# wjf5203/VNext

Hardware: AMD Instinct MI355X
Metric: MSDeformAttn fwd+bwd Gpoints/s (T=5,L=4,Q=300,H=8,K=4) (higher is better)
Workload: dtype f32; 1 GPU; SeqFormer-R50 T=5 360p clip folded to B=5: MSDeformAttn decoder call, Lq=300, S=5100, M=8, D=32, L=4, K=4, loc~U[0,1); 1 step = fwd+bwd; input_rotation_sets=12, parallelism=dp1 (clips sharded, no data-path collective)

## Files before the change

### vnext_amd/csrc/msda_d32_gvdirect_body.h

```cpp
#pragma once
#include <type_traits>

#include "msda_gv_common.h"

namespace vnx {
namespace rec {

#ifndef VNX_GVD_UNITS_PER_CU
#define VNX_GVD_UNITS_PER_CU 3
#endif
#ifndef VNX_GVD_PARTS
#define VNX_GVD_PARTS 2
#endif
#ifndef VNX_GVD_AUX
#define VNX_GVD_AUX 0
#endif
#ifndef VNX_GVD_ABL
#define VNX_GVD_ABL 0
#endif
#ifndef VNX_GVD_FULL_BARRIERS
#define VNX_GVD_FULL_BARRIERS 0
#endif


#ifdef VNX_GVD_STAMPS
static __device__ unsigned long long g_gvd_stamps[4096 * 8];
#define VNX_GVD_STAMP(k) do { if (tid == 0 && vblock < 4096) g_gvd_stamps[vblock * 8 + (k)] = (unsigned long long)wall_clock64(); } while (0)
#else
#define VNX_GVD_STAMP(k) do { } while (0)
#endif

constexpr int kGvdQc = VNX_GVD_QC;
constexpr int kGvdRows = VNX_GVD_ROWS;
constexpr int kGvdSamples = kGvdQc * 4;
constexpr int kGvdSpt = (kGvdSamples + kThreads - 1) / kThreads;
constexpr int kGvdCap = 4 * kGvdSamples;
constexpr int kGvdParts = VNX_GVD_PARTS;
constexpr int kGvdPartPieces = 8 / kGvdParts;
constexpr int kGvdRowPieces = (kGvdQc * kGvdPartPieces + kThreads - 1) / kThreads;
constexpr size_t kGvdLdsBytes = size_t(kGvdQc) * 16 * kGvdPartPieces + size_t(kGvdCap) * 6 + size_t(kGvdRows) * 4 + 16 + 4 * kLevelsMax * 4;
static_assert(kGvdParts == 1 || kGvdParts == 2, "whole rows or halves");
static_assert(kGvdLdsBytes * VNX_GVD_UNITS_PER_CU <= 160 * 1024, "the units that share a CU must fit its LDS");
static_assert(kGvdCap < 65536 && kGvdQc < 65536, "tap ranks and query slots fit 16 bits");

template <typename TV, typename TL, int P_T>
__device__ __forceinline__ void msda_bwd_gv_direct_body(const int64_t* __restrict__ shapes, const int64_t* __restrict__ lsi,
                                                        const TL* __restrict__ loc, const TL* __restrict__ attn,
                                                        const TV* __restrict__ grad_out, TV* __restrict__ grad_value,
                                                        const MsdaDims& d, int ut, int rows_max, int compact, unsigned long long* stamps,
                                                        uint32_t vblock, unsigned char* smem) {
  stamp_begin(stamps);
  constexpr int D = 32;
  float4_t* grows = reinterpret_cast<float4_t*>(smem);
  float* l_wt = reinterpret_cast<float*>(grows + kGvdQc * kGvdPartPieces);
  uint32_t* cnt = reinterpret_cast<uint32_t*>(l_wt + kGvdCap);
  uint32_t* alloc = cnt + kGvdRows;
  int* meta = reinterpret_cast<int*>(alloc + 4);
  uint16_t* l_slot = reinterpret_cast<uint16_t*>(meta + 4 * kLevelsMax);

  const int P = P_T > 0 ? P_T : d.P;
  const int tid = threadIdx.x, lane = tid & 63;
  int rest, b, m;
  if (kGvPair16 && sizeof(TV) == 2 && (d.M & 1) == 0) gv_decode_block<true>(vblock, d.M, d.B, rest, b, m);
  else gv_decode_block<false>(vblock, d.M, d.B, rest, b, m);
  const int unit = rest / d.B;
  VNX_GVD_STAMP(0);

  const TV* go_head = grad_out + (int64_t(b) * d.Lq * d.M + m) * D;
  const uint32_t q_stride = uint32_t(d.M) * uint32_t(D);
  constexpr uint32_t kOutOfRange = 0x80000000u;
  const __amdgpu_buffer_rsrc_t go_src = uniform_rsrc(go_head, uint32_t(d.Lq) * q_stride * uint32_t(sizeof(TV)));
  int qc = kGvdSamples / P;
  qc = qc < kGvdQc ? qc : kGvdQc;
  float4_t pg[kGvdParts][kGvdRowPieces];
  auto request_rows = [&](int q_lo) {
    const int tg = opaque(tid);
#pragma unroll
    for (int part = 0; part < kGvdParts; ++part) {
#pragma unroll
      for (int i = 0; i < kGvdRowPieces; ++i) {
        const int g = i * kThreads + tg, ql = g / kGvdPartPieces;
        const bool ok = ql < qc && q_lo + ql < d.Lq;
        const uint32_t off = ok ? (__umul24(uint32_t(q_lo + ql), q_stride) + uint32_t(part * kGvdPartPieces + g % kGvdPartPieces) * 4u) * uint32_t(sizeof(TV))
                                : kOutOfRange;
        pg[part][i] = load4_buf<TV>(go_src, off);
      }
    }
  };
  auto stage_rows = [&](int part) {
    const int tg = opaque(tid);
#pragma unroll
    for (int i = 0; i < kGvdRowPieces; ++i)
      if ((i * kThreads + tg) / kGvdPartPieces < kGvdQc) grows[i * kThreads + tg] = pg[part][i];
  };
  int lvl = -1, r0 = 0, r1 = 0, Hl = 0, Wl = 0, start = 0, gshift = 0;
  bool packed = true;
  if (tid < d.L) {
    const int H = int(shapes[2 * tid]), W = int(shapes[2 * tid + 1]), first = int(lsi[tid]);
    const GvdSplit sp = gvd_level_split(H * W, ut, d.Lq, P, rows_max);
    meta[4 * tid] = H; meta[4 * tid + 1] = W; meta[4 * tid + 2] = first;
    meta[4 * tid + 3] = sp.units | (sp.rpu << 18) | (sp.gshift << 29);
  }
  for (int i = tid; i < kGvdRows; i += kThreads) cnt[i] = 0;
  if (tid == 0) alloc[0] = 0;
  lds_barrier();
  {
    int running = 0;
    int u = unit;
    for (int l = 0; l < d.L; ++l) {
      packed = packed && (meta[4 * l + 2] == running);
      running += meta[4 * l] * meta[4 * l + 1];
    }
    for (int l = d.L - 1; l >= 0; --l) {
      const int H = meta[4 * l], W = meta[4 * l + 1], st = meta[4 * l + 2];
      const uint32_t ur = uint32_t(meta[4 * l + 3]);
      const int n = H * W, units = int(ur & 0x3ffffu), rpu = int((ur >> 18) & 0x7ffu);
      if (lvl < 0) {
        if (u < units) {
          lvl = l; Hl = H; Wl = W; start = st; gshift = int(ur >> 29);
          r0 = u * rpu;
          r1 = r0 + rpu < n ? r0 + rpu : n;
        } else {
          u -= units;
        }
      }
    }
    packed = packed && (running == d.S);
  }
  if (!packed || lvl < 0) {
    return;
  }
  lvl = __builtin_amdgcn_readfirstlane(lvl); r0 = __builtin_amdgcn_readfirstlane(r0); r1 = __builtin_amdgcn_readfirstlane(r1);
  Hl = __builtin_amdgcn_readfirstlane(Hl); Wl = __builtin_amdgcn_readfirstlane(Wl); start = __builtin_amdgcn_readfirstlane(start);
  gshift = __builtin_amdgcn_readfirstlane(gshift);
  if (VNX_GVD_ABL == 1) { asm volatile("s_waitcnt vmcnt(0)" ::: "memory"); return; }
  const int rows = r1 - r0;
  VNX_GVD_STAMP(1);

  const int LP = d.L * P;
  const int64_t s_base = compact ? ((int64_t(b) * d.M + m) * d.L + lvl) * int64_t(d.Lq) * P
                                 : (int64_t(b) * d.Lq * d.M + m) * LP + lvl * P;
  const TL* attn_bm = attn + s_base;
  const TL* loc_bm = loc + 2 * s_base;
  const uint32_t s_stride = compact ? uint32_t(P) : uint32_t(d.M) * uint32_t(LP);
  const uint32_t n_samp = uint32_t(d.Lq) * s_stride;
  const __amdgpu_buffer_rsrc_t loc_src = uniform_rsrc(loc_bm, n_samp * 2u * uint32_t(sizeof(TL)));
  const __amdgpu_buffer_rsrc_t attn_src = uniform_rsrc(attn_bm, n_samp * uint32_t(sizeof(TL)));
  const float Hf = float(Hl), Wf = float(Wl);
  const int dr[4] = {0, 1, Wl, Wl + 1};
  TV* out = grad_value + ((int64_t(b) * d.S + start + r0) * d.M + m) * D;

  const int n_pass = (d.Lq + qc - 1) / qc;
  const uint32_t gmask = (1u << gshift) - 1u;

  auto do_pass = [&](const int pass, auto single_tag) {
    constexpr bool kSingle = decltype(single_tag)::value;
    const int q_lo = pass * qc;
    float sx[kGvdSpt], sy[kGvdSpt], sa[kGvdSpt];
    uint32_t svalid = 0;
    {
      const int tq = opaque(tid);
#pragma unroll
      for (int j = 0; j < kGvdSpt; ++j) {
        const uint32_t s = uint32_t(j * kThreads + tq);
        const uint32_t ql = P_T == 4 ? (s >> 2) : s / uint32_t(P);
        const uint32_t k = s - ql * uint32_t(P);
        const bool valid = int(ql) < qc && q_lo + int(ql) < d.Lq;
        svalid |= uint32_t(valid) << j;
        const uint32_t si = valid ? __umul24(uint32_t(q_lo) + ql, s_stride) + k : kOutOfRange;
        if constexpr (sizeof(TL) == 4) {
          const uint2_t xy = __builtin_bit_cast(uint2_t, __builtin_amdgcn_raw_buffer_load_b64(loc_src, int(si * 8u), 0, VNX_GVD_AUX));
          sx[j] = __uint_as_float(xy.x); sy[j] = __uint_as_float(xy.y);
          sa[j] = __uint_as_float(__builtin_amdgcn_raw_buffer_load_b32(attn_src, int(si * 4u), 0, VNX_GVD_AUX));
        } else {
          const uint32_t xy = __builtin_amdgcn_raw_buffer_load_b32(loc_src, int(si * 4u), 0, VNX_GVD_AUX);
          const uint32_t a16 = __builtin_amdgcn_raw_buffer_load_b16(attn_src, int(si * 2u), 0, VNX_GVD_AUX);
          sx[j] = to_acc(__builtin_bit_cast(TL, uint16_t(xy & 0xffffu))); sy[j] = to_acc(__builtin_bit_cast(TL, uint16_t(xy >> 16)));
          sa[j] = to_acc(__builtin_bit_cast(TL, uint16_t(a16)));
        }
      }
    }
    request_rows(q_lo);
    if (pass == 0) VNX_GVD_STAMP(2);

    uint32_t mask = 0;
    int row00[kGvdSpt];
    uint32_t rank[kGvdSpt][2];
#pragma unroll
    for (int j = 0; j < kGvdSpt; ++j) {
      row00[j] = 0; rank[j][0] = rank[j][1] = 0u;
      float lh = 0.f, lw = 0.f;
      uint32_t mj = 0;
      if (svalid & (1u << j)) {
        const float h = sy[j] * Hf - 0.5f, w = sx[j] * Wf - 0.5f;
        if (h > -1.f && w > -1.f && h < Hf && w < Wf) {
          const float hf = floorf(h), wf = floorf(w);
          const int h0 = int(hf), w0 = int(wf);
          lh = h - hf; lw = w - wf;
          const bool top = h0 >= 0, bot = h0 + 1 <= Hl - 1, lef = w0 >= 0, rig = w0 + 1 <= Wl - 1;
          const int p00 = h0 * Wl + w0;
          mj = (uint32_t(top && lef && p00 >= r0 && p00 < r1)) |
               (uint32_t(top && rig && p00 + 1 >= r0 && p00 + 1 < r1) << 1) |
               (uint32_t(bot && lef && p00 + Wl >= r0 && p00 + Wl < r1) << 2) |
               (uint32_t(bot && rig && p00 + Wl + 1 >= r0 && p00 + Wl + 1 < r1) << 3);
          row00[j] = p00 - r0;
        }
      }
      sy[j] = lh; sx[j] = lw;
      if (VNX_GVD_ABL == 2) mj = (lh + lw == 12345.f) ? mj : 0u;
#pragma unroll
      for (int t = 0; t < 4; ++t)
        if (mj & (1u << t)) {
          const uint32_t r = __hip_atomic_fetch_add(cnt + row00[j] + dr[t], 1u, __ATOMIC_RELAXED, __HIP_MEMORY_SCOPE_WORKGROUP);
          rank[j][t >> 1] |= r << ((t & 1) * 16);
        }
      mask |= mj << (4 * j);
    }
    if (pass == 0) VNX_GVD_STAMP(3);
    if (VNX_GVD_FULL_BARRIERS) __syncthreads(); else lds_barrier();
    if (pass == 0) VNX_GVD_STAMP(4);

    for (int rb = 0; rb < rows; rb += kThreads) {
      const int r = rb + tid;
      const uint32_t my_cnt = r < rows ? cnt[r] : 0u;
      const uint32_t incl = wave_inclusive_scan(my_cnt);
      const uint32_t wave_total = uint32_t(__builtin_amdgcn_readlane(int(incl), 63));
      uint32_t base = 0;
      if (lane == 0 && wave_total != 0)
        base = __hip_atomic_fetch_add(alloc, wave_total, __ATOMIC_RELAXED, __HIP_MEMORY_SCOPE_WORKGROUP);
      base = uint32_t(__builtin_amdgcn_readfirstlane(int(base)));
      if (r < rows) cnt[r] = my_cnt | ((base + incl - my_cnt) << 16);
    }
    if (VNX_GVD_FULL_BARRIERS) __syncthreads(); else lds_barrier();
    if (pass == 0) VNX_GVD_STAMP(5);

#pragma unroll
    for (int j = 0; j < kGvdSpt; ++j) {
      const uint32_t mj = (mask >> (4 * j)) & 0xfu;
      if (mj) {
        const float lh = sy[j], lw = sx[j], a = sa[j], hh = 1.f - lh, hw = 1.f - lw;
        const float wt[4] = {a * (hh * hw), a * (hh * lw), a * (lh * hw), a * (lh * lw)};
        const uint32_t sj = uint32_t(j * kThreads + opaque(tid));
        const uint32_t slot = P_T == 4 ? (sj >> 2) : sj / uint32_t(P);
#pragma unroll
        for (int t = 0; t < 4; ++t)
          if (mj & (1u << t)) {
            const uint32_t pos = (cnt[row00[j] + dr[t]] >> 16) + ((rank[j][t >> 1] >> ((t & 1) * 16)) & 0xffffu);
            l_slot[pos] = uint16_t(slot);
            l_wt[pos] = wt[t];
          }
      }
    }
    stage_rows(0);
    __syncthreads();
    if (pass == 0) VNX_GVD_STAMP(6);
    if (tid == 0) alloc[0] = 0;

    constexpr int kLpr = 4 / kGvdParts;
    constexpr int kPieces = kGvdPartPieces / kLpr;
    constexpr int kGrp = kThreads / kLpr;
    constexpr int kSlotsMax = kGvdRows > kGvdCap / 8 ? kGvdRows : kGvdCap / 8;
    constexpr int kIters = (kSlotsMax + kGrp - 1) / kGrp;
    static_assert(kIters * kGrp >= kSlotsMax && kSlotsMax >= VNX_GVD_ROWS, "the walk covers every slot gvd_level_split allows");
    float4_t held[kGvdParts == 2 ? kIters : 1][kPieces];
    auto walk = [&](auto cp_tag) {
      constexpr int cp = decltype(cp_tag)::value;
      constexpr bool last = cp == kGvdParts - 1;
      const int ta = opaque(tid);
      const int grp = ta / kLpr, cl = ta % kLpr;
      const uint32_t step = gmask + 1u;
      const int gp = kGvdParts == 2 ? (grp & 1) : 0;
      const float4_t* g4[kPieces];
#pragma unroll
      for (int h = 0; h < kPieces; ++h) g4[h] = grows + cl + kLpr * (h ^ gp);
      const int n_slots = rows << gshift;
#pragma unroll
      for (int it = 0; it < kIters; ++it) {
        const int sb = it * kGrp;
        if (sb >= n_slots) break;
        const int slot = sb + grp;
        const int row = slot >> gshift;
        const uint32_t sub = uint32_t(slot) & gmask;
        uint32_t n = 0, o = 0;
        if (slot < n_slots) {
          const uint32_t w = cnt[row];
          n = VNX_GVD_ABL == 3 ? 0u : (w & 0xffffu); o = w >> 16;
        }
        float4_t a0[kPieces];
#pragma unroll
        for (int h = 0; h < kPieces; ++h) a0[h] = float4_t{0.f, 0.f, 0.f, 0.f};
        uint32_t i = sub;
        for (; i + step < n; i += 2 * step) {
          const uint32_t s0 = l_slot[o + i], s1 = l_slot[o + i + step];
          const float w0 = l_wt[o + i], w1 = l_wt[o + i + step];
          float4_t v0[kPieces], v1[kPieces];
#pragma unroll
          for (int h = 0; h < kPieces; ++h) { v0[h] = g4[h][s0 * kGvdPartPieces]; v1[h] = g4[h][s1 * kGvdPartPieces]; }
#pragma unroll
          for (int h = 0; h < kPieces; ++h) { a0[h] += w0 * v0[h]; a0[h] += w1 * v1[h]; }
        }
        if (i < n) {
          const uint32_t s0 = l_slot[o + i];
          const float w0 = l_wt[o + i];
#pragma unroll
          for (int h = 0; h < kPieces; ++h) a0[h] += w0 * g4[h][s0 * kGvdPartPieces];
        }
#pragma unroll
        for (int sh = 0; sh < 3; ++sh)
          if (sh < gshift) {
            float4_t t[kPieces];
#pragma unroll
            for (int h = 0; h < kPieces; ++h) {
              const float4_t src = a0[(kGvdParts == 2 && sh == 0) ? (h ^ 1) : h];
              t[h].x = __shfl_xor(src.x, kLpr << sh, 64); t[h].y = __shfl_xor(src.y, kLpr << sh, 64);
              t[h].z = __shfl_xor(src.z, kLpr << sh, 64); t[h].w = __shfl_xor(src.w, kLpr << sh, 64);
            }
#pragma unroll
            for (int h = 0; h < kPieces; ++h) a0[h] += t[h];
          }
        if constexpr (!last) {
#pragma unroll
          for (int h = 0; h < kPieces; ++h) held[it][h] = a0[h];
          continue;
        }
        if (VNX_GVD_ABL == 4) continue;
        if constexpr (kGvdParts == 2) {
          if (!kSingle && sub == 0u && slot < n_slots) cnt[row] = 0u;
          const int slot_e = slot & ~1, slot_o = slot | 1;
          const bool ok_e = (uint32_t(slot_e) & gmask) == 0u && slot_e < n_slots;
          const bool ok_o = (uint32_t(slot_o) & gmask) == 0u && slot_o < n_slots;
          const uint32_t lane_el = uint32_t(ta & 3) * 4u;
          TV* pe = out + __umul24(uint32_t(slot_e >> gshift), q_stride) + lane_el;
          TV* po = out + __umul24(uint32_t(slot_o >> gshift), q_stride) + lane_el;
          auto quad_rows = [&](const float4_t first, const float4_t second, float4_t& even_row, float4_t& odd_row) {
            float sx, sy, sz, sw_;
            asm volatile(
                "s_nop 1\n\t"
                "v_mov_b32_dpp %0, %4 quad_perm:[2,3,0,1] row_mask:0xf bank_mask:0xf\n\t"
                "v_mov_b32_dpp %1, %5 quad_perm:[2,3,0,1] row_mask:0xf bank_mask:0xf\n\t"
                "v_mov_b32_dpp %2, %6 quad_perm:[2,3,0,1] row_mask:0xf bank_mask:0xf\n\t"
                "v_mov_b32_dpp %3, %7 quad_perm:[2,3,0,1] row_mask:0xf bank_mask:0xf"
                : "=&v"(sx), "=&v"(sy), "=&v"(sz), "=&v"(sw_)
                : "v"(second.x), "v"(second.y), "v"(second.z), "v"(second.w));
            const float4_t sw = {sx, sy, sz, sw_};
            even_row = gp ? sw : first;
            odd_row = gp ? first : sw;
          };
          float4_t xe[2], xo[2];
          quad_rows(held[it][0], held[it][1], xe[0], xo[0]);
          quad_rows(a0[0], a0[1], xe[1], xo[1]);
          if (ok_e) {
#pragma unroll
            for (int c = 0; c < 2; ++c) {
              if (!kSingle && pass > 0) xe[c] += load4<TV>(pe + c * 16);
              store4<TV>(pe + c * 16, xe[c]);
            }
          }
          if (ok_o) {
#pragma unroll
            for (int c = 0; c < 2; ++c) {
              if (!kSingle && pass > 0) xo[c] += load4<TV>(po + c * 16);
              store4<TV>(po + c * 16, xo[c]);
            }
          }
        } else if (sub == 0u && slot < n_slots) {
          if (!kSingle) cnt[row] = 0u;
          TV* p = out + __umul24(uint32_t(row), q_stride) + cl * 4;
#pragma unroll
          for (int h = 0; h < kPieces; ++h) {
            if (!kSingle && pass > 0) a0[h] += load4<TV>(p + h * kLpr * 4);
            store4<TV>(p + h * kLpr * 4, a0[h]);
          }
        }
      }
    };
    walk(std::integral_constant<int, 0>{});
    if constexpr (kGvdParts == 2) {
      __syncthreads();
      stage_rows(1);
      __syncthreads();
      walk(std::integral_constant<int, 1>{});
    }
    if (!kSingle && pass + 1 < n_pass) __syncthreads();
  };
  if (n_pass == 1) {
    do_pass(0, std::true_type{});
  } else {
    for (int pass = 0; pass < n_pass; ++pass) do_pass(pass, std::false_type{});
  }
  VNX_GVD_STAMP(7);
  stamp_end(stamps);
}


}
}
```

Baseline: 6.902 Gpoints/s.

## Sort grad_value rows by tap count to balance wave work in gather walk

Adds an optional counting sort of value rows by their tap count, binned in LDS, so that rows with similar work land in the same wave during the accumulation walk. Odd iterations use a reversed group mapping, and waves whose lanes all have zero taps skip the inner loop through a ballot. The aim is to cut divergence and idle lanes caused by uneven per-row tap counts, at the cost of extra LDS atomics, a bpermute scan and an indirect row lookup. The path is enabled only when VNX_DEV_VARIANTS is defined and defaults off otherwise.

Result: slower. 6.826 Gpoints/s (-1.1%).

```diff
diff --git a/vnext_amd/csrc/msda_d32_gvdirect_body.h b/vnext_amd/csrc/msda_d32_gvdirect_body.h
--- a/vnext_amd/csrc/msda_d32_gvdirect_body.h
+++ b/vnext_amd/csrc/msda_d32_gvdirect_body.h
@@ -20,6 +20,13 @@
 #endif
 #ifndef VNX_GVD_FULL_BARRIERS
 #define VNX_GVD_FULL_BARRIERS 0
+#endif
+#ifndef VNX_GVD_ORDER
+#ifdef VNX_DEV_VARIANTS
+#define VNX_GVD_ORDER 1
+#else
+#define VNX_GVD_ORDER 0
+#endif
 #endif
 
 
@@ -38,9 +45,14 @@
 constexpr int kGvdParts = VNX_GVD_PARTS;
 constexpr int kGvdPartPieces = 8 / kGvdParts;
 constexpr int kGvdRowPieces = (kGvdQc * kGvdPartPieces + kThreads - 1) / kThreads;
-constexpr size_t kGvdLdsBytes = size_t(kGvdQc) * 16 * kGvdPartPieces + size_t(kGvdCap) * 6 + size_t(kGvdRows) * 4 + 16 + 4 * kLevelsMax * 4;
+constexpr int kGvdOrdBins = 32, kGvdOrdCopies = 2, kGvdOrdWords = kGvdOrdBins * kGvdOrdCopies;
+constexpr size_t kGvdMetaBytes = 4 * kLevelsMax * 4;
+constexpr size_t kGvdOrdTableBytes = VNX_GVD_ORDER && size_t(kGvdRows) * 2 > kGvdMetaBytes ? size_t(kGvdRows) * 2 : kGvdMetaBytes;
+constexpr size_t kGvdOrdBytes = (VNX_GVD_ORDER ? size_t(kGvdOrdWords) * 4 : 0) + kGvdOrdTableBytes - kGvdMetaBytes;
+static_assert(kGvdOrdWords == 64 && kGvdRows <= 2 * kThreads && kGvdRows <= 1024, "one bin word per lane; a thread packs two rows' (word, rank) in 32 bits");
+constexpr size_t kGvdLdsBytes = size_t(kGvdQc) * 16 * kGvdPartPieces + size_t(kGvdCap) * 6 + size_t(kGvdRows) * 4 + 16 + 4 * kLevelsMax * 4 + kGvdOrdBytes;
 static_assert(kGvdParts == 1 || kGvdParts == 2, "whole rows or halves");
-static_assert(kGvdLdsBytes * VNX_GVD_UNITS_PER_CU <= 160 * 1024, "the units that share a CU must fit its LDS");
+static_assert((kGvdLdsBytes + 1279) / 1280 * 1280 * VNX_GVD_UNITS_PER_CU <= 160 * 1024, "the units that share a CU must fit its LDS");
 static_assert(kGvdCap < 65536 && kGvdQc < 65536, "tap ranks and query slots fit 16 bits");
 
 template <typename TV, typename TL, int P_T>
@@ -56,7 +68,9 @@
   uint32_t* cnt = reinterpret_cast<uint32_t*>(l_wt + kGvdCap);
   uint32_t* alloc = cnt + kGvdRows;
   int* meta = reinterpret_cast<int*>(alloc + 4);
-  uint16_t* l_slot = reinterpret_cast<uint16_t*>(meta + 4 * kLevelsMax);
+  uint16_t* order = reinterpret_cast<uint16_t*>(meta);
+  uint16_t* l_slot = reinterpret_cast<uint16_t*>(reinterpret_cast<unsigned char*>(meta) + kGvdOrdTableBytes);
+  uint32_t* obins = reinterpret_cast<uint32_t*>(l_slot + kGvdCap);
 
   const int P = P_T > 0 ? P_T : d.P;
   const int tid = threadIdx.x, lane = tid & 63;
@@ -103,6 +117,7 @@
   }
   for (int i = tid; i < kGvdRows; i += kThreads) cnt[i] = 0;
   if (tid == 0) alloc[0] = 0;
+  if (VNX_GVD_ORDER && tid < kGvdOrdWords) obins[tid] = 0;
   lds_barrier();
   {
     int running = 0;
@@ -220,9 +235,16 @@
     if (VNX_GVD_FULL_BARRIERS) __syncthreads(); else lds_barrier();
     if (pass == 0) VNX_GVD_STAMP(4);
 
+    uint32_t ordw = 0;
     for (int rb = 0; rb < rows; rb += kThreads) {
       const int r = rb + tid;
       const uint32_t my_cnt = r < rows ? cnt[r] : 0u;
+      if (VNX_GVD_ORDER && r < rows) {
+        const uint32_t key = (my_cnt >> gshift) < uint32_t(kGvdOrdBins - 1) ? (my_cnt >> gshift) : uint32_t(kGvdOrdBins - 1);
+        const uint32_t e = key * kGvdOrdCopies + (uint32_t(lane) & uint32_t(kGvdOrdCopies - 1));
+        const uint32_t rk = __hip_atomic_fetch_add(obins + e, 1u, __ATOMIC_RELAXED, __HIP_MEMORY_SCOPE_WORKGROUP);
+        ordw |= (e | (rk << 6)) << (rb ? 16 : 0);
+      }
       const uint32_t incl = wave_inclusive_scan(my_cnt);
       const uint32_t wave_total = uint32_t(__builtin_amdgcn_readlane(int(incl), 63));
       uint32_t base = 0;
@@ -233,6 +255,7 @@
     }
     if (VNX_GVD_FULL_BARRIERS) __syncthreads(); else lds_barrier();
     if (pass == 0) VNX_GVD_STAMP(5);
+    const uint32_t obin = VNX_GVD_ORDER ? obins[lane] : 0u;
 
 #pragma unroll
     for (int j = 0; j < kGvdSpt; ++j) {
@@ -251,10 +274,19 @@
           }
       }
     }
+    if (VNX_GVD_ORDER) {
+      const uint32_t first = wave_inclusive_scan(obin) - obin;
+      for (int rb = 0; rb < rows; rb += kThreads) {
+        const uint32_t w = (ordw >> (rb ? 16 : 0)) & 0xffffu;
+        const uint32_t pos = uint32_t(__builtin_amdgcn_ds_bpermute(int((w & 63u) << 2), int(first))) + (w >> 6);
+        if (rb + tid < rows) order[pos] = uint16_t(rb + tid);
+      }
+    }
     stage_rows(0);
     __syncthreads();
     if (pass == 0) VNX_GVD_STAMP(6);
     if (tid == 0) alloc[0] = 0;
+    if (VNX_GVD_ORDER && !kSingle && tid < kGvdOrdWords) obins[tid] = 0;
 
     constexpr int kLpr = 4 / kGvdParts;
     constexpr int kPieces = kGvdPartPieces / kLpr;
@@ -278,18 +310,19 @@
       for (int it = 0; it < kIters; ++it) {
         const int sb = it * kGrp;
         if (sb >= n_slots) break;
-        const int slot = sb + grp;
-        const int row = slot >> gshift;
+        const int slot = sb + ((VNX_GVD_ORDER && (it & 1)) ? (grp ^ ((kGrp - 1) & ~31)) : grp);
+        auto row_at = [&](int sl) { return VNX_GVD_ORDER ? int(order[sl >> gshift]) : sl >> gshift; };
         const uint32_t sub = uint32_t(slot) & gmask;
         uint32_t n = 0, o = 0;
         if (slot < n_slots) {
-          const uint32_t w = cnt[row];
+          const uint32_t w = cnt[row_at(slot)];
           n = VNX_GVD_ABL == 3 ? 0u : (w & 0xffffu); o = w >> 16;
         }
         float4_t a0[kPieces];
 #pragma unroll
         for (int h = 0; h < kPieces; ++h) a0[h] = float4_t{0.f, 0.f, 0.f, 0.f};
         uint32_t i = sub;
+        if (!VNX_GVD_ORDER || __builtin_amdgcn_ballot_w64(i < n) != 0) {
         for (; i + step < n; i += 2 * step) {
           const uint32_t s0 = l_slot[o + i], s1 = l_slot[o + i + step];
           const float w0 = l_wt[o + i], w1 = l_wt[o + i + step];
@@ -304,6 +337,7 @@
           const float w0 = l_wt[o + i];
 #pragma unroll
           for (int h = 0; h < kPieces; ++h) a0[h] += w0 * g4[h][s0 * kGvdPartPieces];
+        }
         }
 #pragma unroll
         for (int sh = 0; sh < 3; ++sh)
@@ -325,13 +359,14 @@
         }
         if (VNX_GVD_ABL == 4) continue;
         if constexpr (kGvdParts == 2) {
-          if (!kSingle && sub == 0u && slot < n_slots) cnt[row] = 0u;
           const int slot_e = slot & ~1, slot_o = slot | 1;
+          const int row_e = row_at(slot_e), row_o = row_at(slot_o);
+          if (!kSingle && sub == 0u && slot < n_slots) cnt[gp ? row_o : row_e] = 0u;
           const bool ok_e = (uint32_t(slot_e) & gmask) == 0u && slot_e < n_slots;
           const bool ok_o = (uint32_t(slot_o) & gmask) == 0u && slot_o < n_slots;
           const uint32_t lane_el = uint32_t(ta & 3) * 4u;
-          TV* pe = out + __umul24(uint32_t(slot_e >> gshift), q_stride) + lane_el;
-          TV* po = out + __umul24(uint32_t(slot_o >> gshift), q_stride) + lane_el;
+          TV* pe = out + __umul24(uint32_t(row_e), q_stride) + lane_el;
+          TV* po = out + __umul24(uint32_t(row_o), q_stride) + lane_el;
           auto quad_rows = [&](const float4_t first, const float4_t second, float4_t& even_row, float4_t& odd_row) {
             float sx, sy, sz, sw_;
             asm volatile(
@@ -364,6 +399,7 @@
             }
           }
         } else if (sub == 0u && slot < n_slots) {
+          const int row = row_at(slot);
           if (!kSingle) cnt[row] = 0u;
           TV* p = out + __umul24(uint32_t(row), q_stride) + cl * 4;
 #pragma unroll
```
